# RamSaw/PipelineDP

Hardware: AMD Instinct MI355X
Metric: records/sec DPEngine.aggregate COUNT+SUM at 1/2/4/8 MI355X; % HBM roofline (higher is better)
Workload: dtype f64; 1 GPU; configs[1]: 1e+09 records / 1e+07 privacy ids / 1e+06 Zipf(1.1) partitions per GPU, COUNT+SUM+PRIVACY_ID_COUNT, private partition selection; records_per_gpu=1000000000, privacy_ids_per_gpu=10000000, partitions=1000000, max_partitions_contributed=8, max_contributions_per_partition=2, noise=laplace, selection=truncated_geometric, parallelism=pid-sharded x1, privacy_id_range_supplied=True

## Files before the change

pipelinedp_amd/csrc/dpg_api.hip:

```cpp
#include <dlfcn.h>
#include <hip/hip_runtime.h>
#include <rccl/rccl.h>

#include <algorithm>
#include <cstddef>
#include <chrono>
#include <cmath>
#include <cstdio>
#include <cstdlib>
#include <cstring>
#include <map>
#include <mutex>
#include <string>
#include <thread>
#include <tuple>
#include <vector>

static hipError_t occ_query(int *blocks, const void *kern, int threads, size_t lds) {
    static std::mutex mu;
    static std::map<std::tuple<int, const void *, int, size_t>, int> cache;
    int dev = 0;
    (void)hipGetDevice(&dev);
    std::lock_guard<std::mutex> g(mu);
    const auto key = std::make_tuple(dev, kern, threads, lds);
    const auto it = cache.find(key);
    if (it != cache.end()) {
        *blocks = it->second;
        return hipSuccess;
    }
    const hipError_t e = hipOccupancyMaxActiveBlocksPerMultiprocessor(blocks, kern, threads, lds);
    if (e == hipSuccess) cache[key] = *blocks;
    return e;
}
static hipError_t set_func_attr(const void *kern, hipFuncAttribute attr, int value) {
    if (attr != hipFuncAttributeMaxDynamicSharedMemorySize) return hipFuncSetAttribute(kern, attr, value);
    static std::mutex mu;
    static std::map<std::pair<int, const void *>, int> done;
    int dev = 0;
    (void)hipGetDevice(&dev);
    std::lock_guard<std::mutex> g(mu);
    const auto key = std::make_pair(dev, kern);
    const auto it = done.find(key);
    if (it != done.end() && it->second >= value) return hipSuccess;
    const hipError_t e = hipFuncSetAttribute(kern, attr, value);
    if (e == hipSuccess) done[key] = value;
    return e;
}

#include "dpg_bound.h"
#include "dpg_chunk.h"
#include "dpg_common.h"
#include "dpg_hist.h"
#include "dpg_keydict.h"
#include "dpg_owner.h"
#include "dpg_pairx.h"
#include "dpg_partition.h"
#include "dpg_quantile.h"
#include "dpg_records.h"
#include "dpg_rsort.h"
#include "dpg_sample.h"
#include "dpg_select.h"
#include "dpg_shard.h"
#include "dpg_sortb.h"
#include "dpg_sortmw.h"
#include "dpg_team.h"
#include "dpg_utility.h"
#include "dpg_vsum.h"
#include "dpg_wave.h"
#include "dpg_hist_phases.h"

using namespace dpg;

namespace {

constexpr uint32_t kBucketTarget = 256;
constexpr uint32_t kMaxB1 = 11, kMaxB2 = 12, kMaxBR = 11;
constexpr uint32_t kMaxB1W = 12;
constexpr int kIptL1W = 8;
constexpr uint32_t kPinErr = 4096;
constexpr uint32_t kChunkGroup = 32;
constexpr int kRedoLevel2 = -100;
#ifndef DPG_PC_HALF
#define DPG_PC_HALF 0
#endif
#ifndef DPG_IPT_PC
#define DPG_IPT_PC 8
#endif

struct Buf {
    void *p = nullptr;
    size_t bytes = 0;
};

struct Control {
    uint32_t err;
    uint32_t item_cursor;
    uint32_t ntiles[8];
    int64_t n_scalar;
    uint32_t n_chunks;
    uint32_t n_over;
    uint32_t n_over2;
    uint32_t n_mchunks;
    uint32_t heavy_nfb;
    uint32_t pad_;
    unsigned long long over_records;
    unsigned long long over2_records;
    unsigned long long pid_lo, pid_hi;
};

}

struct dpg_ctx {
    int device = 0;
    uint64_t seed = 0;
    int n_cu = 256;
    std::string err;
    std::map<std::string, Buf> bufs;
    std::vector<std::string> stage_names;
    std::vector<hipEvent_t> events;
    int n_events_used = 0;
    hipStream_t last_stream = nullptr;
    uint32_t bucket_target = 0;
    uint32_t bucket_cap = kBCap;
    void *comm = nullptr;
    const uint32_t *last_err = nullptr;
    int rank = 0, nranks = 1;
    char *stage_buf = nullptr;
    size_t stage_cap = 0, stage_head = 0;
    std::map<hipStream_t, hipEvent_t> stage_done;
    uint32_t *pin_tot = nullptr;
    hipEvent_t tot_ev = nullptr;
    uint32_t team_backoff = 0;
    uint32_t team_backoff_next = 64;
};

namespace {

int watchdog_seconds() {
#if defined(DPG_WATCHDOG) || defined(DPG_PHASE_TIMING)
    const char *e = std::getenv("DPG_WATCHDOG_S");
    return e ? std::atoi(e) : 0;
#else
    return 0;
#endif
}

uint32_t *watchdog_buffer(size_t n) {
    static uint32_t *buf = nullptr;
    static size_t cap = 0;
    if (n > cap) {
        if (buf) (void)hipHostFree(buf);
        if (hipHostMalloc((void **)&buf, n * 4, hipHostMallocCoherent) != hipSuccess) return nullptr;
        cap = n;
    }
    std::memset(buf, 0, n * 4);
    return buf;
}

void watchdog_wait(hipStream_t s, const uint32_t *prog, size_t n, const char *what) {
    int secs = watchdog_seconds();
    for (int i = 0; i < secs * 100; ++i) {
        if (hipStreamQuery(s) == hipSuccess) return;
        std::this_thread::sleep_for(std::chrono::milliseconds(10));
    }
    std::fprintf(stderr, "[dpg watchdog] %s did not finish in %d s; phases:", what, secs);
    for (size_t i = 0; i < n; ++i) std::fprintf(stderr, " %u", prog[i]);
    std::fprintf(stderr, "\n");
    std::fflush(stderr);
    std::abort();
}

int fail(dpg_ctx *c, int code, const std::string &msg) {
    if (c) c->err = msg;
    return code;
}

#define HIP_TRY(expr)                                                                     \
    do {                                                                                  \
        hipError_t e_ = (expr);                                                           \
        if (e_ != hipSuccess)                                                             \
            return fail(ctx, DPG_ERR_HIP, std::string(#expr) + ": " + hipGetErrorString(e_)); \
    } while (0)

#define LAUNCH_CHECK()                                                                        \
    do {                                                                                      \
        hipError_t e_ = hipGetLastError();                                                    \
        if (e_ != hipSuccess)                                                                 \
// ... 779 lines not shown
            for (uint8_t x : hd) nd += x;
            std::fprintf(stderr, "[dpg phase] medium chunks streamed=%u deferred=%zu\n",
                         hctl.n_mchunks, nd);
        }
    }
    if (heavy) {
        HIP_TRY(hipMemcpyAsync(&hctl, ctl, sizeof(Control), hipMemcpyDeviceToHost, s));
        HIP_TRY(hipStreamSynchronize(s));
        const uint32_t nfb = hctl.heavy_nfb;
        if (nfb > 0) {
            WS(fst, int64_t, "heavy.fb.start", nfb);
            WS(fcnt, uint32_t, "heavy.fb.cnt", nfb);
            WS(fd1, uint32_t, "heavy.fb.d1", nfb);
            k_gather_heavy<<<(nfb + 255) / 256, 256, 0, s>>>(hfb, &ctl->heavy_nfb, g_start, g_cnt,
                                                             g_d1, fst, fcnt, fd1);
            LAUNCH_CHECK();
            g_start = fst;
            g_cnt = fcnt;
            g_d1 = fd1;
        }
        if (timing) std::fprintf(stderr, "[dpg phase] heavy buckets=%u handed back=%u\n", n_global, nfb);
        n_global = nfb;
    }
    if (n_global > 0) {
        std::vector<uint32_t> cnt(n_global);
        HIP_TRY(hipMemcpy(cnt.data(), g_cnt, n_global * 4, hipMemcpyDeviceToHost));
        std::vector<size_t> off(n_global);
        size_t total = 0;
        for (uint32_t i = 0; i < n_global; ++i) {
            off[i] = total;
            total += align16(BigLayout::make(cnt[i], ItemTraits<Item>::var).total);
        }
        WS(scratch, char, "bound.scratch", total);
        WS(doff, size_t, "bound.scratch_off", n_global);
        UPLOAD(doff, off.data(), n_global * sizeof(size_t));
        BoundParams bpg = bp;
        uint32_t *gprog = watchdog_seconds() ? watchdog_buffer(n_global) : nullptr;
        bpg.progress = gprog;
        bpg.phase_cyc = timing ? bpl.phase_cyc + 32 : nullptr;
        if (watchdog_seconds())
            std::fprintf(stderr, "[dpg] %u oversize buckets, scratch %zu bytes\n", n_global, total);
        k_bound_big<Item, R><<<n_global, kBigThreads, 0, s>>>(g_base, g_start, g_cnt, g_d1, doff,
                                                              scratch, bpg, items, wg_off + G,
                                                              wg_cnt + G);
        LAUNCH_CHECK();
        if (gprog) watchdog_wait(s, gprog, n_global, "k_bound_big");
        if (timing) {
            unsigned long long h[8];
            HIP_TRY(hipMemcpy(h, bpl.phase_cyc + 32, sizeof(h), hipMemcpyDeviceToHost));
            static const char *nmb[8] = {"clear", "A.insert", "B.slots", "C.mpc", "D.state",
                                         "E.mcpp", "F.acc", "G.emit"};
            unsigned long long tot = 0;
            for (int i = 0; i < 8; ++i) tot += h[i];
            size_t recs_big = 0;
            uint32_t nmax = 0;
            for (uint32_t i = 0; i < n_global; ++i) recs_big += cnt[i], nmax = std::max(nmax, cnt[i]);
            std::fprintf(stderr, "[dpg phase] big buckets=%u records=%zu max=%u per-WG Mcycles:",
                         n_global, recs_big, nmax);
            for (int i = 0; i < 8; ++i)
                std::fprintf(stderr, " %s=%.3f(%.0f%%)", nmb[i], h[i] / 1e6 / n_global,
                             100.0 * h[i] / (tot ? tot : 1));
            std::fprintf(stderr, "\n");
        }
    }
    k_scan_small<<<1, 1024, 0, s>>>(wg_cnt, G + 1, wg_pre, &ctl->item_cursor);
    LAUNCH_CHECK();
    constexpr bool kPA = ItemTraits<Item>::preagg;
    int64_t n_items;
    if constexpr (kPA) {
        HIP_TRY(hipMemcpyAsync(&hctl, ctl, sizeof(Control), hipMemcpyDeviceToHost, s));
        HIP_TRY(hipStreamSynchronize(s));
        if (hctl.err & 2u) return fail(ctx, DPG_ERR_HIP, "internal hash-table error in bounding");
        n_items = hctl.item_cursor;
    } else {
        const uint64_t pairs_per_id = std::max<uint32_t>(1u, per_pid ? bp.L : bp.mpc);
        n_items = (int64_t)std::min<uint64_t>((uint64_t)items_cap,
                                              ((uint64_t)1 << pl.kbits) * pairs_per_id);
    }
    const int64_t P = pl.P;
#ifndef DPG_ITEM_IPT_WIDE
#define DPG_ITEM_IPT_WIDE 4
#endif
    constexpr int kItemIpt = sizeof(Item) == 16 ? 8 : sizeof(Item) == 24 ? DPG_ITEM_IPT_WIDE : 4;
#ifndef DPG_PA_RB
#define DPG_PA_RB 11
#endif
    constexpr uint32_t kRB = kPA ? (uint32_t)DPG_PA_RB : (uint32_t)kRangeBits;
    const int64_t nranges = (P + (1ll << kRB) - 1) >> kRB;
    int64_t *baseR = nullptr;
    uint32_t *totR = nullptr;
    const Item *sorted = items;
    uint32_t F = 1;
    if (n_items > 0) {
        const uint32_t rb = std::max<uint32_t>(1, bits_for((uint64_t)std::max<int64_t>(1, nranges)));
        const uint32_t b2 = rb > 10 ? std::min<uint32_t>(kMaxBR, rb / 2) : 0u;
        const uint32_t b1 = rb - b2;
        const uint32_t F1 = nranges <= 1024 ? (uint32_t)std::max<int64_t>(1, nranges) : 1u << b1;
        WS(items2, Item, "items2", n_items);
        const SrcSeg<Item> src1{items, wg_pre, wg_off, G + 1, kRB + b2};
        int r = run_level<SrcSeg<Item>, Item, kItemIpt, 1024>(
            ctx, s, src1, 1u, nullptr, &ctl->item_cursor, nullptr, n_items, F1, b1, items2,
            "items", &baseR, &totR, &ctl->ntiles[4]);
        if (r) return r;
        sorted = items2;
        F = F1;
        if (b2 > 0) {
            const SrcItems<Item> src2{items2, kRB, (1u << b2) - 1u};
            int64_t *base2;
            uint32_t *tot2;
            r = run_level<SrcItems<Item>, Item, kItemIpt, 2048>(ctx, s, src2, F1, baseR, totR,
                                                                 nullptr, n_items, 1u << b2, b2,
                                                                 items, "items2", &base2, &tot2,
                                                                 &ctl->ntiles[6]);
            if (r) return r;
            baseR = base2;
            totR = tot2;
            sorted = items;
            F = F1 << b2;
        }
    }
    if constexpr (kPA) {
        pa->n_pairs = n_items;
        if (n_items > pa->capacity)
            return fail(ctx, DPG_ERR_INVALID_ARG,
                        "pairs capacity " + std::to_string(pa->capacity) + " < " +
                            std::to_string(n_items) + " pairs");
        if (n_items == 0) {
            HIP_TRY(hipMemsetAsync(pa->partition_start, 0, (P + 1) * 8, s));
            stage(ctx, s, "end");
            return DPG_OK;
        }
        const SrcItems<Item> src3{sorted, 0u, (1u << kRB) - 1u};
        int64_t *base3;
        uint32_t *tot3;
        int r = run_level<SrcItems<Item>, Item, kItemIpt, 2048>(
            ctx, s, src3, F, baseR, totR, nullptr, n_items, 1u << kRB, kRB, pa->pairs, "pairs",
            &base3, &tot3, &ctl->ntiles[7]);
        if (r) return r;
        HIP_TRY(hipMemcpyAsync(pa->partition_start, base3, P * 8, hipMemcpyDeviceToDevice, s));
        k_set_i64<<<1, 1, 0, s>>>(pa->partition_start + P, n_items);
        LAUNCH_CHECK();
    } else if (n_items > 0) {
        Partials po{out->rows, out->count, out->sum, out->nsum, out->nsq};
        stage(ctx, s, "reduce");
        const int64_t rtile = 65536;
        uint32_t max_tiles = (uint32_t)(n_items / rtile + F + 1);
        WS(rt, TileDesc, "reduce.tiles", max_tiles);
        WS(rstb, uint32_t, "reduce.stb", F);
        WS(rsnt, uint32_t, "reduce.snt", F);
        k_build_tiles<<<build_tiles_blocks(F), 256, 0, s>>>(baseR, totR, nullptr, F, rtile, rt, rstb,
                                                      rsnt, &ctl->ntiles[5]);
        LAUNCH_CHECK();
        size_t lds_r = (size_t)kRange * 8 * (ItemTraits<Item>::var ? (ItemTraits<Item>::sum ? 3 : 2) : 1) +
                       kRange * 8;
        k_reduce_items<Item><<<max_tiles, 1024, lds_r, s>>>(sorted, rt, &ctl->ntiles[5], rsnt, P,
                                                         po);
        LAUNCH_CHECK();
    }
    stage(ctx, s, "end");
    return DPG_OK;
}

__global__ void k_region_base(int64_t *rbase, uint32_t F, uint32_t C) {
    const uint32_t i = blockIdx.x * blockDim.x + threadIdx.x;
    if (i >= 8 * F) return;
    const uint32_t x = i / F, d = i % F;
    rbase[i] = ((int64_t)d * 8 + x) * C;
}

__global__ __launch_bounds__(1024) void k_piece_totals(const uint32_t *cum, const int64_t *rbase,
                                                       uint32_t F, uint32_t *tot, uint32_t *ptot,
                                                       int64_t *ostart, PieceDesc *desc) {
    __shared__ uint32_t sh[16];
    constexpr int DPT = 4;
    const uint32_t d0 = DPT * threadIdx.x;
    uint32_t c[DPT], x = 0;
#pragma unroll
    for (int u = 0; u < DPT; ++u) {
        c[u] = 0;
        uint32_t cp = 0;
        if (d0 + u < F) {
            const uint32_t d = d0 + u;
            const int64_t b0 = rbase[d];
            PieceDesc &pd = desc[d];
            for (int r = 0; r < 8; ++r) {
                const uint32_t y = cum[(size_t)r * F + d];
// ... 2181 lines not shown
```

pipelinedp_amd/csrc/dpg_partition.h:

```cpp
#pragma once

#include "dpg_common.h"

#include <type_traits>

namespace dpg {

#ifndef DPG_HIST_U
#define DPG_HIST_U 8
#endif
#ifndef DPG_SCAT_WB
#define DPG_SCAT_WB 2
#endif
constexpr int kPartThreads = 1024;
constexpr int kScatThreads = 1024;

__host__ __device__ constexpr size_t a16(size_t x) { return (x + 15) & ~(size_t)15; }

typedef int64_t i64x2 __attribute__((ext_vector_type(2)));
typedef uint64_t u64x2 __attribute__((ext_vector_type(2)));
typedef uint64_t u64x2a8 __attribute__((ext_vector_type(2), aligned(8)));

template <class Src, class = void>
struct HasFetchPairs {
    static constexpr bool value = false;
};
template <class Src>
struct HasFetchPairs<Src, decltype((void)Src::kFetchPairs)> {
    static constexpr bool value = Src::kFetchPairs;
};

#ifndef DPG_XTILE_PF
#define DPG_XTILE_PF 1
#endif
template <class Src, class = void>
struct HasTilePrefetch {
    static constexpr bool value = false;
};
template <class Src>
struct HasTilePrefetch<Src, decltype((void)Src::kTilePrefetch)> {
    static constexpr bool value = Src::kTilePrefetch && DPG_XTILE_PF;
};

template <class Src, class = void>
struct HasPieces {
    static constexpr bool value = false;
};
template <class Src>
struct HasPieces<Src, decltype((void)Src::kPieces)> {
    static constexpr bool value = Src::kPieces;
};

template <class Src, class = void>
struct HasPairs {
    static constexpr bool value = false;
};
template <class Src>
struct HasPairs<Src, decltype((void)Src::kPairs)> {
    static constexpr bool value = Src::kPairs;
};

struct TileDesc {
    int64_t begin, end;
    uint32_t seg;
    uint32_t pad;
};

__device__ __forceinline__ TileDesc uniform_tile(const TileDesc *tiles, uint32_t t) {
    const TileDesc d = tiles[t];
    auto u64 = [](int64_t x) {
        return (int64_t)(((uint64_t)__builtin_amdgcn_readfirstlane((uint32_t)((uint64_t)x >> 32)) << 32) |
                         (uint32_t)__builtin_amdgcn_readfirstlane((uint32_t)x));
    };
    TileDesc r;
    r.begin = u64(d.begin);
    r.end = u64(d.end);
    r.seg = __builtin_amdgcn_readfirstlane(d.seg);
    r.pad = __builtin_amdgcn_readfirstlane(d.pad);
    return r;
}

template <class R, bool kFull = false>
struct SrcSoAKey {
    static constexpr bool kDigitFromRec = false;
    static constexpr bool kTilePrefetch = true;
    static constexpr bool kPieces = kFull;
    static constexpr bool kV = sizeof(R) == 16;
    using PidW = std::conditional_t<kFull, uint64_t, uint32_t>;
    struct RawK {
        PidW pid;
        int64_t pk;
    };
    struct RawV {
        PidW pid;
        int64_t pk;
        double v;
    };
    using Raw = std::conditional_t<kV, RawV, RawK>;
    const int64_t *pid;
    const int64_t *pk;
    const uint8_t *pub;
    int64_t P;
    int64_t pid_min;
    uint64_t U;
// ... 68 lines not shown
#endif
    static constexpr bool kFetchPairs = DPG_L1_PAIRS != 0;
    __device__ __forceinline__ void fetch2(int64_t i, Raw &x0, Raw &x1) const {
#if DPG_L1_NT
        const u64x2a8 p = __builtin_nontemporal_load(reinterpret_cast<const u64x2a8 *>(pid + i));
        const u64x2a8 q = __builtin_nontemporal_load(reinterpret_cast<const u64x2a8 *>(pk + i));
#else
        const u64x2a8 p = *reinterpret_cast<const u64x2a8 *>(pid + i);
        const u64x2a8 q = *reinterpret_cast<const u64x2a8 *>(pk + i);
#endif
        if constexpr (kV) {
#if DPG_L1_NT
            const u64x2a8 v = __builtin_nontemporal_load(reinterpret_cast<const u64x2a8 *>(value + i));
#else
            const u64x2a8 v = *reinterpret_cast<const u64x2a8 *>(value + i);
#endif
            x0 = Raw{(PidW)p.x, (int64_t)q.x, __builtin_bit_cast(double, v.x)};
            x1 = Raw{(PidW)p.y, (int64_t)q.y, __builtin_bit_cast(double, v.y)};
        } else {
            x0 = Raw{(PidW)p.x, (int64_t)q.x};
            x1 = Raw{(PidW)p.y, (int64_t)q.y};
        }
    }
    static constexpr bool kPairs = true;
    __device__ __forceinline__ bool pairs_ok() const {
        return ((uintptr_t)pid & 15) == 0 && (!pub || ((uintptr_t)pk & 15) == 0);
    }
    __device__ __forceinline__ void hist2(int64_t i, uint32_t (&d)[2], bool (&ok)[2]) const {
        const i64x2 p = *reinterpret_cast<const i64x2 *>(pid + i);
        const uint64_t a0 = (uint64_t)(p.x - pid_min), a1 = (uint64_t)(p.y - pid_min);
        if (a0 >= U || a1 >= U) atomicOr(err, 1u);
        d[0] = hk((uint32_t)a0, H) >> dshift;
        d[1] = hk((uint32_t)a1, H) >> dshift;
        ok[0] = ok[1] = true;
        if (pub) {
            const i64x2 q = *reinterpret_cast<const i64x2 *>(pk + i);
            ok[0] = keep((uint32_t)a0, q.x);
            ok[1] = keep((uint32_t)a1, q.y);
        }
    }
};

template <class R>
struct SrcAoS {
    static constexpr bool kDigitFromRec = true;
    static constexpr bool kTilePrefetch = true;
    using Raw = R;
    const R *a;
    Fmt f;
    uint32_t shift, mask;
    __device__ __forceinline__ R fetch(int64_t i) const { return a[i]; }
    __device__ __forceinline__ uint32_t digit(const R &r) const {
        return (uint32_t)(RecOps<R>::key(r, f) >> shift) & mask;
    }
    __device__ __forceinline__ bool decode(const R &x, int64_t, R &r, uint32_t &d) const {
        r = x;
        d = digit(x);
        return true;
    }
    __device__ __forceinline__ bool hist(int64_t i, uint32_t &d) const {
        d = digit(a[i]);
        return true;
    }
    static constexpr bool kPairs = sizeof(R) == 8;
    static constexpr bool kFetchPairs = sizeof(R) == 8;
    __device__ __forceinline__ void fetch2(int64_t i, R &x0, R &x1) const {
        if constexpr (sizeof(R) == 8) {
            const u64x2a8 w = *reinterpret_cast<const u64x2a8 *>(a + i);
            x0 = R{w.x};
            x1 = R{w.y};
        }
    }
    __device__ __forceinline__ bool pairs_ok() const { return ((uintptr_t)a & 15) == 0; }
    __device__ __forceinline__ void hist2(int64_t i, uint32_t (&d)[2], bool (&ok)[2]) const {
        if constexpr (sizeof(R) == 8) {
            const u64x2 w = *reinterpret_cast<const u64x2 *>(a + i);
            d[0] = digit(R{w.x});
            d[1] = digit(R{w.y});
        }
        ok[0] = ok[1] = true;
    }
};

template <class T>
struct SrcSeg {
    static constexpr bool kDigitFromRec = true;
    using Raw = T;
    const T *a;
    const int64_t *pre;
    const int64_t *off;
    uint32_t S;
    uint32_t shift;
    int64_t lo = 0, hi = 0, base = 0;
    __device__ __forceinline__ T fetch(int64_t i) {
        if (i < lo || i >= hi) {
            uint32_t l = 0, h = S;
            while (h - l > 1) {
                const uint32_t mid = (l + h) >> 1;
                if (pre[mid] <= i) l = mid;
                else h = mid;
            }
            lo = pre[l];
            hi = pre[l + 1];
            base = off[l] - lo;
        }
        return a[base + i];
    }
    __device__ __forceinline__ uint32_t digit(const T &r) const { return r.pk >> shift; }
    __device__ __forceinline__ bool decode(const T &x, int64_t, T &r, uint32_t &d) const {
        r = x;
        d = digit(x);
        return true;
    }
    __device__ __forceinline__ bool hist(int64_t i, uint32_t &d) {
        d = digit(fetch(i));
        return true;
    }
};

template <class T>
struct SrcItems {
    static constexpr bool kDigitFromRec = true;
    using Raw = T;
    const T *a;
    uint32_t shift, mask;
    __device__ __forceinline__ T fetch(int64_t i) const { return a[i]; }
    __device__ __forceinline__ uint32_t digit(const T &r) const { return (r.pk >> shift) & mask; }
    __device__ __forceinline__ bool decode(const T &x, int64_t, T &r, uint32_t &d) const {
        r = x;
        d = digit(x);
        return true;
    }
    __device__ __forceinline__ bool hist(int64_t i, uint32_t &d) const {
        d = digit(a[i]);
        return true;
    }
};

struct XcdQueues {
    uint32_t *q;
    uint32_t *n;
    uint32_t *next;
    uint32_t stride;
};

__global__ void k_build_tiles_single(int64_t n, int64_t tile, uint32_t G, TileDesc *tiles,
                                     uint32_t *seg_tile_base, uint32_t *seg_ntiles,
                                     uint32_t *ntiles_total, XcdQueues xq) {
    const uint32_t nt = (uint32_t)((n + tile - 1) / tile);
    const uint32_t t = blockIdx.x * blockDim.x + threadIdx.x;
    if (t == 0) {
        seg_tile_base[0] = 0;
        seg_ntiles[0] = nt;
        *ntiles_total = nt;
    }
    if (t >= nt) return;
    TileDesc d;
    d.begin = (int64_t)t * tile;
    d.end = min((int64_t)(t + 1) * tile, n);
    d.seg = 0;
    d.pad = 0;
    tiles[t] = d;
    if (!xq.q) return;
    const uint32_t g = t / G, x = g & 7u;
    xq.q[(size_t)x * xq.stride + (g >> 3) * G + t % G] = t;
    atomicAdd(&xq.n[x], 1u);
}

__global__ void k_build_subtiles(const TileDesc *groups, const uint32_t *ngroups, int64_t sub,
                                 TileDesc *tiles, uint32_t *ntiles_total, XcdQueues xq) {
    const uint32_t g = blockIdx.x * blockDim.x + threadIdx.x;
    if (g >= *ngroups) return;
    const TileDesc gd = groups[g];
    const uint32_t nt = (uint32_t)((gd.end - gd.begin + sub - 1) / sub);
    if (!nt) return;
    const uint32_t b = atomicAdd(ntiles_total, nt);
    for (uint32_t j = 0; j < nt; ++j) {
        TileDesc d;
        d.begin = gd.begin + (int64_t)j * sub;
        d.end = min(gd.begin + (int64_t)(j + 1) * sub, gd.end);
        d.seg = gd.seg;
        d.pad = g;
        tiles[b + j] = d;
    }
    const uint32_t x = g & 7u;
    const uint32_t qb = atomicAdd(&xq.n[x], nt);
    for (uint32_t j = 0; j < nt; ++j) xq.q[(size_t)x * xq.stride + qb + j] = b + j;
}

__global__ __launch_bounds__(256) void k_build_tiles(const int64_t *seg_start,
                                                     const uint32_t *seg_cnt,
// ... 8 lines not shown
    if (s >= S) return;
    const int64_t st = seg_start ? seg_start[s] : 0;
    const int64_t n = seg_cnt64 ? seg_cnt64[s] : (int64_t)seg_cnt[s];
    const uint32_t nt = (uint32_t)((n + tile - 1) / tile);
    const uint32_t x = s & 7u;
    uint32_t b = 0, qb = 0;
    if (lane == 0 && nt) {
        b = atomicAdd(ntiles_total, nt);
        if (xq.q) qb = atomicAdd(&xq.n[x], nt);
    }
    b = (uint32_t)__shfl((int)b, 0, 64);
    qb = (uint32_t)__shfl((int)qb, 0, 64);
    if (lane == 0) {
        seg_tile_base[s] = b;
        seg_ntiles[s] = nt;
    }
    for (uint32_t j = lane; j < nt; j += 64) {
        TileDesc d;
        d.begin = st + (int64_t)j * tile;
        d.end = st + min((int64_t)(j + 1) * tile, n);
        d.seg = s;
        d.pad = 0;
        tiles[b + j] = d;
        if (xq.q) xq.q[(size_t)x * xq.stride + qb + j] = b + j;
    }
}

inline uint32_t build_tiles_blocks(uint32_t S) { return (S + 3) / 4; }

template <class Src>
__global__ __launch_bounds__(kPartThreads) void k_hist(Src src_in, const TileDesc *tiles,
                                                       const uint32_t *ntiles, uint32_t F,
                                                       uint32_t *hist) {
    extern __shared__ __attribute__((aligned(16))) uint32_t lh[];
    const uint32_t t = blockIdx.x;
    if (t >= *ntiles) return;
    const TileDesc td = tiles[t];
    const int tid = threadIdx.x;
    const uint32_t copy = (tid >> 6) & 3;
    for (uint32_t d = tid; d < 4 * F; d += kPartThreads) lh[d] = 0;
    __syncthreads();
    uint32_t *my = lh + copy * F;
    Src src = src_in;
    constexpr int U = DPG_HIST_U;
    if constexpr (HasPairs<Src>::value) {
        if (src.pairs_ok()) {
            int64_t b = td.begin;
            const int64_t e = td.end;
            if (b & 1) {
                uint32_t d;
                if (tid == 0 && b < e && src.hist(b, d)) atomicAdd(&my[d], 1u);
                ++b;
            }
            constexpr int U2 = U / 2 > 0 ? U / 2 : 1;
            int64_t i = b + 2 * tid;
            for (; i + 2 * (U2 - 1) * kPartThreads + 1 < e; i += 2 * U2 * kPartThreads) {
                uint32_t d[U2][2];
                bool ok[U2][2];
#pragma unroll
                for (int u = 0; u < U2; ++u) src.hist2(i + 2 * u * kPartThreads, d[u], ok[u]);
#pragma unroll
                for (int u = 0; u < U2; ++u) {
                    if (ok[u][0]) atomicAdd(&my[d[u][0]], 1u);
                    if (ok[u][1]) atomicAdd(&my[d[u][1]], 1u);
                }
            }
            for (; i + 1 < e; i += 2 * kPartThreads) {
                uint32_t d[2];
                bool ok[2];
                src.hist2(i, d, ok);
                if (ok[0]) atomicAdd(&my[d[0]], 1u);
                if (ok[1]) atomicAdd(&my[d[1]], 1u);
            }
            if (i < e) {
                uint32_t d;
                if (src.hist(i, d)) atomicAdd(&my[d], 1u);
            }
            __syncthreads();
            for (uint32_t d = tid; d < F; d += kPartThreads)
                hist[(size_t)t * F + d] = lh[d] + lh[F + d] + lh[2 * F + d] + lh[3 * F + d];
            return;
        }
    }
    int64_t i = td.begin + tid;
    for (; i + (U - 1) * kPartThreads < td.end; i += U * kPartThreads) {
        uint32_t d[U];
        bool ok[U];
#pragma unroll
        for (int u = 0; u < U; ++u) ok[u] = src.hist(i + u * kPartThreads, d[u]);
#pragma unroll
        for (int u = 0; u < U; ++u)
            if (ok[u]) atomicAdd(&my[d[u]], 1u);
    }
    for (; i < td.end; i += kPartThreads) {
        uint32_t d;
        if (src.hist(i, d)) atomicAdd(&my[d], 1u);
    }
    __syncthreads();
    for (uint32_t d = tid; d < F; d += kPartThreads)
        hist[(size_t)t * F + d] = lh[d] + lh[F + d] + lh[2 * F + d] + lh[3 * F + d];
}

__global__ __launch_bounds__(1024) void k_scan_tiles(const uint32_t *seg_tile_base,
                                                     const uint32_t *seg_ntiles, uint32_t F,
                                                     uint32_t *hist, uint32_t *ctot) {
    __shared__ uint32_t part[16][64];
    const uint32_t s = blockIdx.x, c = blockIdx.z, C = gridDim.z;
    const int lane = threadIdx.x & 63, w = threadIdx.x >> 6;
    const uint32_t d = blockIdx.y * 64 + lane;
    const uint32_t nt_all = seg_ntiles[s];
    const uint32_t per = (nt_all + C - 1) / C;
    const uint32_t c0 = min(nt_all, c * per), c1 = min(nt_all, c0 + per);
    const uint32_t nt = c1 - c0, tb = seg_tile_base[s] + c0;
    const uint32_t ch = (nt + 15) / 16;
    const uint32_t t0 = min(nt, w * ch), t1 = min(nt, (w + 1) * ch);
    uint32_t acc = 0;
    if (d < F)
        for (uint32_t t = t0; t < t1; ++t) acc += hist[(size_t)(tb + t) * F + d];
    part[w][lane] = acc;
    __syncthreads();
    uint32_t pre = 0, total = 0;
    for (int k = 0; k < 16; ++k) {
        uint32_t x = part[k][lane];
        if (k < w) pre += x;
        total += x;
    }
    if (d < F) {
        uint32_t run = pre;
        for (uint32_t t = t0; t < t1; ++t) {
            size_t o = (size_t)(tb + t) * F + d;
            uint32_t x = hist[o];
            hist[o] = run;
            run += x;
        }
        if (w == 0) ctot[((size_t)s * C + c) * F + d] = total;
    }
}

__global__ void k_scan_chunks(uint32_t S, uint32_t C, uint32_t F, uint32_t *ctot, uint32_t *tot) {
    const uint32_t i = blockIdx.x * blockDim.x + threadIdx.x;
    if (i >= S * F) return;
    const uint32_t s = i / F, d = i % F;
    uint32_t run = 0;
    for (uint32_t c = 0; c < C; ++c) {
        uint32_t &x = ctot[((size_t)s * C + c) * F + d];
        const uint32_t v = x;
        x = run;
        run += v;
    }
    tot[(size_t)s * F + d] = run;
}

__device__ __forceinline__ uint32_t block_excl_scan_1024(uint32_t x, uint32_t *sh16,
                                                         uint32_t &total) {
    const int lane = threadIdx.x & 63, w = threadIdx.x >> 6;
    uint32_t wt;
    uint32_t e = wave_excl_scan(x, wt);
    if (lane == 63) sh16[w] = wt;
    __syncthreads();
    uint32_t pre = 0, tot = 0;
    for (int k = 0; k < 16; ++k) {
        uint32_t y = sh16[k];
        if (k < w) pre += y;
        tot += y;
    }
    __syncthreads();
// ... 240 lines not shown
        uint64_t bal = __ballot((d >> b) & 1u);
        peers &= ((d >> b) & 1u) ? bal : ~bal;
    }
    const int lane = __lane_id();
    const int leader = peers ? __ffsll((long long)peers) - 1 : lane;
    const uint32_t below = __popcll(peers & ((1ull << lane) - 1ull));
    uint32_t basev = 0;
    if (ok && lane == leader) basev = atomicAdd(&cnt[d], (uint32_t)__popcll(peers));
    basev = __shfl(basev, leader, 64);
    return basev + below;
}

template <class T, int kW = (sizeof(T) % 16 == 0 ? 16 : sizeof(T) % 8 == 0 ? 8 : 4)>
struct Words {
    static constexpr int N = sizeof(T) / 16;
    uint4 w[N];
};
template <class T>
struct Words<T, 8> {
    static constexpr int N = sizeof(T) / 8;
    uint2 w[N];
};
template <class T>
struct Words<T, 4> {
    static constexpr int N = sizeof(T) / 4;
    uint32_t w[N];
};
template <class T>
__device__ __forceinline__ Words<T> to_words(const T &r) {
    Words<T> x;
    __builtin_memcpy(&x, &r, sizeof(T));
    return x;
}
template <class T>
__device__ __forceinline__ T from_words(const Words<T> &x) {
    T r;
    __builtin_memcpy(&r, &x, sizeof(T));
    return r;
}

template <class Src, class Rec, int IPT, int FMAX, int NT = kScatThreads>
constexpr size_t scatter_lds_core() {
    return (size_t)sizeof(Rec) * (NT * IPT + 1) +
           (Src::kDigitFromRec ? 0 : a16((size_t)2 * (NT * IPT + 1))) +
           (size_t)FMAX * 12 + 80;
}
#ifndef DPG_SCAT_LBASE
#define DPG_SCAT_LBASE 1
#endif
#ifndef DPG_PC_NORESET
#define DPG_PC_NORESET 1
#endif
#ifndef DPG_PC_LATE_RSV
#define DPG_PC_LATE_RSV 1
#endif
#ifndef DPG_L1_PF
#define DPG_L1_PF 2
#endif
template <class Src, class Rec, int IPT, int FMAX, int NT = kScatThreads>
constexpr bool scatter_lbase() {
    return scatter_lds_core<Src, Rec, IPT, FMAX, NT>() + (size_t)FMAX * 4 <= 160 * 1024;
}
template <class Src, class Rec, int IPT, int FMAX, int NT = kScatThreads>
constexpr size_t scatter_lds() {
    return scatter_lds_core<Src, Rec, IPT, FMAX, NT>() +
           (scatter_lbase<Src, Rec, IPT, FMAX, NT>() ? (size_t)FMAX * 4 : 0);
}

#ifdef DPG_PHASE_TIMING
__device__ unsigned long long g_scat_cyc[8];
#define DPG_SCAT_MARK(k)                                         \
    do {                                                         \
        if (threadIdx.x == 0) {                                  \
            const uint64_t now_ = __builtin_amdgcn_s_memtime();  \
            scyc[k] += now_ - slast;                             \
            slast = now_;                                        \
        }                                                        \
    } while (0)
#else
#define DPG_SCAT_MARK(k) \
    do {                 \
    } while (0)
#endif

template <class T>
__device__ __forceinline__ const T *uniform_ptr(const T *p) {
    const uint64_t v = (uint64_t)(uintptr_t)p;
    const uint32_t lo = __builtin_amdgcn_readfirstlane((uint32_t)v);
    const uint32_t hi = __builtin_amdgcn_readfirstlane((uint32_t)(v >> 32));
    return reinterpret_cast<const T *>((uintptr_t)(((uint64_t)hi << 32) | lo));
}

template <class Src, class Rec, int IPT, int FMAX, bool kAgg, int NT = kScatThreads>
__global__ __launch_bounds__(NT, 4) void k_scatter(Src src_in, const TileDesc *tiles,
                                                          const uint32_t *ntiles, uint32_t F,
                                                          uint32_t bits, const uint32_t *off,
                                                          const int64_t *base, Rec *out,
                                                          XcdQueues xq = XcdQueues{},
                                                          const uint32_t *cbase = nullptr,
                                                          const uint32_t *seg_tile_base = nullptr,
                                                          const uint32_t *seg_ntiles = nullptr,
                                                          uint32_t C = 1, uint32_t *goff = nullptr,
                                                          uint32_t pcap = 0, uint32_t pdump = 0,
                                                          uint32_t *perr = nullptr) {
    constexpr int SUB = NT * IPT;
    constexpr bool kPc = HasPieces<Src>::value;
    constexpr bool kSD = !Src::kDigitFromRec;
    constexpr bool kP = HasFetchPairs<Src>::value && IPT % 2 == 0;
    constexpr bool kEarly = kPc && kP && DPG_L1_PF != 0;
    constexpr int kPF = kEarly ? DPG_L1_PF : 0;
    using W = Words<Rec>;
    extern __shared__ __attribute__((aligned(16))) char smem[];
    W *stage = reinterpret_cast<W *>(smem);
    uint16_t *sdig = reinterpret_cast<uint16_t *>(smem + sizeof(Rec) * (SUB + 1));
    const size_t o = sizeof(Rec) * (SUB + 1) + (kSD ? a16((size_t)2 * (SUB + 1)) : 0);
    uint32_t *cnt = reinterpret_cast<uint32_t *>(smem + o);
    uint32_t *dstart = cnt + FMAX;
    uint32_t *cur = dstart + FMAX + 1;
    uint32_t *sh16 = cur + FMAX;
    constexpr bool kLB = DPG_SCAT_LBASE && scatter_lbase<Src, Rec, IPT, FMAX, NT>();
    uint32_t *lbase = reinterpret_cast<uint32_t *>(smem + scatter_lds_core<Src, Rec, IPT, FMAX, NT>());
    uint32_t lseg = 0xFFFFFFFFu;

    const uint32_t nt = __builtin_amdgcn_readfirstlane(*ntiles);
    const int tid = threadIdx.x;
    auto elem = [tid](int j) -> uint32_t {
        return kP ? (uint32_t)((j >> 1) * 2 * NT + 2 * tid + (j & 1))
                  : (uint32_t)(j * NT + tid);
    };
    __shared__ uint32_t sh_next;
    const uint32_t xq_id = blockIdx.x & 7u;
    const uint32_t xq_len = xq.q ? __builtin_amdgcn_readfirstlane(xq.n[xq_id]) : 0u;
    constexpr uint32_t kNone = 0xFFFFFFFFu;
    Src src = src_in;
    typename Src::Raw raw[IPT];
    auto load_sub = [&](int64_t b0, uint32_t lim) {
        if constexpr (kEarly) {
#pragma unroll
            for (int m = 0; m < IPT / 2; ++m) {
                const int32_t o = m * 2 * NT + 2 * tid;
                src.fetch2(b0 + min(o, (int32_t)lim - 2), raw[2 * m], raw[2 * m + 1]);
            }
            return;
        } else if constexpr (kP) {
            if (lim >= 2) {
#pragma unroll
                for (int m = 0; m < IPT / 2; ++m) {
                    const uint32_t o = m * 2 * NT + 2 * tid;
                    const uint32_t a = min(o, lim - 2);
                    typename Src::Raw x0, x1;
                    src.fetch2(b0 + a, x0, x1);
                    raw[2 * m] = a == o ? x0 : x1;
                    raw[2 * m + 1] = x1;
                }
                return;
            }
        }
#pragma unroll
        for (int j = 0; j < IPT; ++j) raw[j] = src.fetch(b0 + min(elem(j), lim - 1));
    };
    auto decode_raw = [&](int j, uint32_t lim, int64_t i, Rec &r, uint32_t &d) -> bool {
        if constexpr (kEarly) {
            if ((j & 1) == 0)
                return src.decode((int32_t)elem(j) > (int32_t)lim - 2 ? raw[j + 1] : raw[j], i, r, d);
        }
        return src.decode(raw[j], i, r, d);
    };
    uint32_t it = blockIdx.x;
    uint32_t t = kNone;
    if (xq.q) {
        if (tid == 0) sh_next = atomicAdd(&xq.next[xq_id], 1u);
        __syncthreads();
        const uint32_t w = __builtin_amdgcn_readfirstlane(sh_next);
        if (w < xq_len) t = __builtin_amdgcn_readfirstlane(xq.q[(size_t)xq_id * xq.stride + w]);
    } else if (it < nt) {
        t = it;
    }
    if (t == kNone) return;
#ifdef DPG_PHASE_TIMING
    uint64_t scyc[6] = {0, 0, 0, 0, 0, 0};
    uint64_t slast = __builtin_amdgcn_s_memtime();
#endif
    TileDesc td = uniform_tile(tiles, t);
    const int64_t n_end = kPc ? uniform_tile(tiles, nt - 1).end : 0;
    load_sub(td.begin, (uint32_t)min<int64_t>(SUB, td.end - td.begin));
    constexpr bool kPcLB = kPc && kLB && DPG_PC_NORESET;
    if constexpr (kPcLB) {
        for (uint32_t d = tid; d < F; d += NT) {
            lbase[d] = (uint32_t)base[(size_t)(blockIdx.x & 7u) * F + d];
            cnt[d] = 0;
        }
        __syncthreads();
    }
    for (;;) {
    uint32_t nq = 0;
    const uint32_t *cb = nullptr;
    uint32_t *gof = goff ? goff + (size_t)(kPc ? (blockIdx.x & 7u) : td.pad) * F : nullptr;
    if constexpr (!kPcLB) {
    if (xq.q && tid == 0) nq = atomicAdd(&xq.next[xq_id], 1u);
    __syncthreads();
    if (cbase) {
        const uint32_t nta = seg_ntiles[td.seg], per = (nta + C - 1) / C;
        cb = cbase + ((size_t)td.seg * C + (t - seg_tile_base[td.seg]) / per) * F;
    }
    const uint32_t bsel = kPc ? (blockIdx.x & 7u) : td.seg;
    if (kLB && goff) {
        if (bsel != lseg) {
            for (uint32_t d = tid; d < F; d += NT) lbase[d] = (uint32_t)base[(size_t)bsel * F + d];
            lseg = bsel;
        }
        for (uint32_t d = tid; d < F; d += NT) {
            cur[d] = lbase[d];
            cnt[d] = 0;
        }
    } else {
        for (uint32_t d = tid; d < F; d += NT) {
            cur[d] = (uint32_t)(base[(size_t)bsel * F + d] +
                                (goff ? 0u : off[(size_t)t * F + d] + (cb ? cb[d] : 0u)));
            cnt[d] = 0;
        }
    }
    __syncthreads();
    }
    uint32_t tn = kNone;
    TileDesc tdn = td;
    DPG_SCAT_MARK(4);
    for (int64_t sb = td.begin; sb < td.end; sb += SUB) {
        const uint32_t lim = (uint32_t)min<int64_t>(SUB, td.end - sb);
        Rec rec[IPT];
        uint32_t dr[IPT];
        if constexpr (!kAgg) {
            uint32_t dg[IPT];
            bool okv[IPT];
#pragma unroll
            for (int j = 0; j < IPT; ++j) {
                const uint32_t o = elem(j);
                uint32_t d = 0;
                if constexpr (kEarly)
                    okv[j] = o < lim && decode_raw(j, lim, sb + o, rec[j], d);
                else
                    okv[j] = o < lim && src.decode(raw[j], sb + o, rec[j], d);
                dg[j] = okv[j] ? d : 0u;
            }
            uint32_t rk[IPT];
#pragma unroll
            for (int j = 0; j < IPT; ++j) rk[j] = atomicAdd(&cnt[dg[j]], okv[j] ? 1u : 0u);
#pragma unroll
            for (int j = 0; j < IPT; ++j) dr[j] = okv[j] ? (dg[j] | (rk[j] << 12)) : ~0u;
        } else {
#pragma unroll
            for (int j = 0; j < IPT; ++j) {
                const uint32_t o = elem(j);
                uint32_t d = 0;
                bool ok;
                if constexpr (kEarly)
                    ok = o < lim && decode_raw(j, lim, sb + o, rec[j], d);
                else
                    ok = o < lim && src.decode(raw[j], sb + o, rec[j], d);
                const uint32_t rk = wave_agg_rank(cnt, ok ? d : 0u, ok, bits);
                dr[j] = ok ? (d | (rk << 12)) : ~0u;
            }
        }
        if (xq.q && tid == 0 && sb == td.begin) sh_next = nq;
        __syncthreads();
        DPG_SCAT_MARK(0);
        constexpr int kDPT = FMAX / NT;
        constexpr bool kLate = kPcLB && (kDPT == 2 || kDPT == 4) && FMAX == kDPT * NT && DPG_PC_LATE_RSV;
        PcRsv<(kDPT >= 2 ? kDPT : 2)> rsv;
        uint32_t total;
        if constexpr (!kEarly) {
        if constexpr (kLate)
            total = scatter_scan_pc<NT, kDPT>(cnt, dstart, F, sh16, gof, rsv);
        else
            total = scatter_scan_update<NT, FMAX / NT, kPc>(
                cnt, dstart, cur, F, sh16, gof, pcap, pdump, perr, kPcLB ? lbase : nullptr);
        DPG_SCAT_MARK(1);
        {
            uint32_t ds[IPT];
#pragma unroll
            for (int j = 0; j < IPT; ++j) ds[j] = dstart[dr[j] != ~0u ? (dr[j] & 0xFFFu) : 0u];
#pragma unroll
            for (int j = 0; j < IPT; ++j) {
                const uint32_t pos = dr[j] != ~0u ? ds[j] + (dr[j] >> 12) : (uint32_t)SUB;
                stage[pos] = to_words(rec[j]);
                if constexpr (kSD) sdig[pos] = (uint16_t)(dr[j] & 0xFFFu);
            }
        }
        if constexpr (kLate) scatter_rsv_finish(rsv, cur, lbase, F, pcap, pdump, perr);
        __syncthreads();
        DPG_SCAT_MARK(2);
        const int64_t nb = sb + SUB;
        const uint32_t nlim = (uint32_t)max<int64_t>(0, min<int64_t>(SUB, td.end - nb));
        {
            int64_t lb = nb;
            uint32_t ll = nlim;
            if constexpr (HasTilePrefetch<Src>::value && kPc) {
                if (nlim == 0 && it + gridDim.x < nt) {
                    tn = it + gridDim.x;
                    tdn.begin = (int64_t)tn * SUB;
                    tdn.end = min(tdn.begin + SUB, n_end);
                    lb = tdn.begin;
                    ll = (uint32_t)min<int64_t>(SUB, tdn.end - tdn.begin);
                }
            } else if constexpr (HasTilePrefetch<Src>::value) {
                if (nlim == 0 && xq.q) {
                    const uint32_t w = __builtin_amdgcn_readfirstlane(sh_next);
                    if (w < xq_len) {
                        tn = __builtin_amdgcn_readfirstlane(xq.q[(size_t)xq_id * xq.stride + w]);
                        tdn = uniform_tile(tiles, tn);
                        lb = tdn.begin;
                        ll = (uint32_t)min<int64_t>(SUB, tdn.end - tdn.begin);
                    }
                }
            }
            if (ll > 0) load_sub(lb, ll);
        }
        } else {
        auto prefetch = [&]() {
            const int64_t nb = sb + SUB;
            const uint32_t nlim = (uint32_t)max<int64_t>(0, min<int64_t>(SUB, td.end - nb));
            int64_t lb = nb;
            uint32_t ll = nlim;
            if (nlim == 0) {
                lb = sb;
                ll = lim;
                if (it + gridDim.x < nt) {
                    tn = it + gridDim.x;
                    tdn.begin = (int64_t)tn * SUB;
                    tdn.end = min(tdn.begin + SUB, n_end);
                    lb = tdn.begin;
                    ll = (uint32_t)min<int64_t>(SUB, tdn.end - tdn.begin);
                }
            }
            load_sub(lb, ll);
        };
        if constexpr (kLate && kPF == 3) {
            total = scatter_scan_pc<NT, kDPT>(cnt, dstart, F, sh16, gof, rsv, prefetch);
        } else {
            if constexpr (kLate)
                total = scatter_scan_pc<NT, kDPT>(cnt, dstart, F, sh16, gof, rsv);
            else
                total = scatter_scan_update<NT, FMAX / NT, kPc>(
                    cnt, dstart, cur, F, sh16, gof, pcap, pdump, perr, kPcLB ? lbase : nullptr);
            prefetch();
        }
        DPG_SCAT_MARK(1);
        {
            uint32_t ds[IPT];
#pragma unroll
            for (int j = 0; j < IPT; ++j) ds[j] = dstart[dr[j] != ~0u ? (dr[j] & 0xFFFu) : 0u];
#pragma unroll
            for (int j = 0; j < IPT; ++j) {
                const uint32_t pos = dr[j] != ~0u ? ds[j] + (dr[j] >> 12) : (uint32_t)SUB;
                stage[pos] = to_words(rec[j]);
                if constexpr (kSD) sdig[pos] = (uint16_t)(dr[j] & 0xFFFu);
            }
        }
        if constexpr (kLate) scatter_rsv_finish(rsv, cur, lbase, F, pcap, pdump, perr);
        __syncthreads();
        DPG_SCAT_MARK(2);
        }
        constexpr int WB = IPT < DPG_SCAT_WB ? IPT : DPG_SCAT_WB;
        constexpr int kWbIter = (IPT + WB - 1) / WB;
        auto write_batch = [&](uint32_t k0) {
            W x[WB];
            uint32_t dd[WB], kc[WB];
#pragma unroll
            for (int u = 0; u < WB; ++u) {
                kc[u] = min(k0 + u * NT + tid, total - 1);
                x[u] = stage[kc[u]];
                if constexpr (kSD) dd[u] = sdig[kc[u]];
            }
            if constexpr (!kSD) {
#pragma unroll
                for (int u = 0; u < WB; ++u) dd[u] = src.digit(from_words<Rec>(x[u]));
            }
            uint32_t c1[WB], c2[WB];
#pragma unroll
            for (int u = 0; u < WB; ++u) {
                c1[u] = cur[dd[u]];
                c2[u] = dstart[dd[u] + 1];
            }
#if DPG_EXP_SCAT_NOSTORE
#pragma unroll
            for (int u = 0; u < WB; ++u) {
                uint32_t w0;
                __builtin_memcpy(&w0, &x[u], 4);
                if (w0 == 0x12345u && c1[u] == 0x777u)
                    *reinterpret_cast<W *>(&out[c1[u] - c2[u] + kc[u]]) = x[u];
            }
#else
#pragma unroll
            for (int u = 0; u < WB; ++u) *reinterpret_cast<W *>(&out[c1[u] - c2[u] + kc[u]]) = x[u];
#endif
        };
        if constexpr (kPc) {
#pragma unroll
            for (int b = 0; b < kWbIter; ++b) {
                if ((uint32_t)b * WB * NT >= total) break;
                write_batch((uint32_t)b * WB * NT);
            }
        } else {
            for (uint32_t k0 = 0; k0 < total; k0 += WB * NT) write_batch(k0);
        }
        DPG_SCAT_MARK(3);
#ifdef DPG_PHASE_TIMING
        if (tid == 0) ++scyc[5];
#endif
    }
    if (!HasTilePrefetch<Src>::value && xq.q) {
        const uint32_t w = __builtin_amdgcn_readfirstlane(sh_next);
        if (w >= xq_len) break;
        tn = __builtin_amdgcn_readfirstlane(xq.q[(size_t)xq_id * xq.stride + w]);
        tdn = uniform_tile(tiles, tn);
        load_sub(tdn.begin, (uint32_t)min<int64_t>(SUB, tdn.end - tdn.begin));
    } else if (kPc && HasTilePrefetch<Src>::value) {
        it += gridDim.x;
    } else if (!xq.q) {
        it += gridDim.x;
        if (it >= nt) break;
        tn = it;
        tdn = uniform_tile(tiles, tn);
        load_sub(tdn.begin, (uint32_t)min<int64_t>(SUB, tdn.end - tdn.begin));
    }
    if (tn == kNone) break;
    t = tn;
    td = tdn;
    }
#ifdef DPG_PHASE_TIMING
    if (tid == 0)
        for (int k = 0; k < 6; ++k) atomicAdd(&g_scat_cyc[k], (unsigned long long)scyc[k]);
#endif
}

}
```

Measured before the change: 56.47 billion records/s.

## Resolve segmented item regions per sub-tile with scalar-loaded window and lane permute

Replaces the per-element binary search in SrcSeg fetch with a per-subtile window: the wave finds the starting region with a ballot-based parallel search, scalar-loads eight region bounds and offsets, and each lane picks its base address through a bpermute. This applies to both the histogram and scatter passes of the first items sort level, with a fallback to the old per-element fetch when the window does not cover the subtile. It also changes the items IPT for 16-byte items to 5 and reads and writes staged items as raw vector words in the scatter writeback. The cost it targets is the divergent per-element region lookup. In exchange it adds inline asm, a per-subtile atomic path counter, and a requirement of at least eight regions.

```diff
diff --git a/pipelinedp_amd/csrc/dpg_api.hip b/pipelinedp_amd/csrc/dpg_api.hip
--- a/pipelinedp_amd/csrc/dpg_api.hip
+++ b/pipelinedp_amd/csrc/dpg_api.hip
@@ -103,6 +103,7 @@
     uint32_t n_mchunks;
     uint32_t heavy_nfb;
     uint32_t pad_;
+    uint32_t seg_paths[2];
     unsigned long long over_records;
     unsigned long long over2_records;
     unsigned long long pid_lo, pid_hi;
@@ -1048,6 +1049,10 @@
 #define DPG_ITEM_IPT_WIDE 4
 #endif
     constexpr int kItemIpt = sizeof(Item) == 16 ? 8 : sizeof(Item) == 24 ? DPG_ITEM_IPT_WIDE : 4;
+#ifndef DPG_ITEM_IPT_SEG16
+#define DPG_ITEM_IPT_SEG16 5
+#endif
+    constexpr int kSegIpt = sizeof(Item) == 16 ? DPG_ITEM_IPT_SEG16 : kItemIpt;
 #ifndef DPG_PA_RB
 #define DPG_PA_RB 11
 #endif
@@ -1063,11 +1068,19 @@
         const uint32_t b1 = rb - b2;
         const uint32_t F1 = nranges <= 1024 ? (uint32_t)std::max<int64_t>(1, nranges) : 1u << b1;
         WS(items2, Item, "items2", n_items);
-        const SrcSeg<Item> src1{items, wg_pre, wg_off, G + 1, kRB + b2};
-        int r = run_level<SrcSeg<Item>, Item, kItemIpt, 1024>(
+        if (G + 1 < (uint32_t)kSegK) return fail(ctx, DPG_ERR_HIP, "internal: too few item regions");
+        const SrcSeg<Item> src1{items, wg_pre, wg_off, G + 1, kRB + b2, ctl->seg_paths};
+        int r = run_level<SrcSeg<Item>, Item, kSegIpt, 1024>(
             ctx, s, src1, 1u, nullptr, &ctl->item_cursor, nullptr, n_items, F1, b1, items2,
             "items", &baseR, &totR, &ctl->ntiles[4]);
         if (r) return r;
+        if (std::getenv("DPG_DEBUG_ITEM_PATHS")) {
+            uint32_t hp[2];
+            HIP_TRY(hipMemcpyAsync(hp, ctl->seg_paths, sizeof(hp), hipMemcpyDeviceToHost, s));
+            HIP_TRY(hipStreamSynchronize(s));
+            if (hp[0]) stage(ctx, s, "items.regions=window");
+            if (hp[1]) stage(ctx, s, "items.regions=lookup");
+        }
         sorted = items2;
         F = F1;
         if (b2 > 0) {
diff --git a/pipelinedp_amd/csrc/dpg_partition.h b/pipelinedp_amd/csrc/dpg_partition.h
--- a/pipelinedp_amd/csrc/dpg_partition.h
+++ b/pipelinedp_amd/csrc/dpg_partition.h
@@ -20,6 +20,8 @@
 typedef int64_t i64x2 __attribute__((ext_vector_type(2)));
 typedef uint64_t u64x2 __attribute__((ext_vector_type(2)));
 typedef uint64_t u64x2a8 __attribute__((ext_vector_type(2), aligned(8)));
+typedef uint32_t u32x2 __attribute__((ext_vector_type(2)));
+typedef uint32_t u32x4 __attribute__((ext_vector_type(4)));
 
 template <class Src, class = void>
 struct HasFetchPairs {
@@ -254,16 +256,163 @@
     }
 };
 
+template <class Src, class = void>
+struct HasRegions {
+    static constexpr bool value = false;
+};
+template <class Src>
+struct HasRegions<Src, decltype((void)Src::kRegions)> {
+    static constexpr bool value = Src::kRegions;
+};
+
+constexpr int kSegK = 8;
+
+template <class T>
+__device__ __forceinline__ const T *uniform_ptr(const T *p) {
+    const uint64_t v = (uint64_t)(uintptr_t)p;
+    const uint32_t lo = __builtin_amdgcn_readfirstlane((uint32_t)v);
+    const uint32_t hi = __builtin_amdgcn_readfirstlane((uint32_t)(v >> 32));
+    return reinterpret_cast<const T *>((uintptr_t)(((uint64_t)hi << 32) | lo));
+}
+
+struct SegBounds {
+    int64_t p0, p1, p2, p3, p4, p5, p6, p7, p8;
+    int64_t o0, o1, o2, o3, o4, o5, o6, o7;
+};
+__device__ __forceinline__ SegBounds sload_regions(const int64_t *pre, const int64_t *off) {
+    static_assert(kSegK == 8, "sload_regions lists its loads");
+    int64_t p0, p1, p2, p3, p4, p5, p6, p7, p8, o0, o1, o2, o3, o4, o5, o6, o7;
+    asm volatile(
+        "s_load_dwordx2 %0, %17, 0x0\n\t"
+        "s_load_dwordx2 %1, %17, 0x8\n\t"
+        "s_load_dwordx2 %2, %17, 0x10\n\t"
+        "s_load_dwordx2 %3, %17, 0x18\n\t"
+        "s_load_dwordx2 %4, %17, 0x20\n\t"
+        "s_load_dwordx2 %5, %17, 0x28\n\t"
+        "s_load_dwordx2 %6, %17, 0x30\n\t"
+        "s_load_dwordx2 %7, %17, 0x38\n\t"
+        "s_load_dwordx2 %8, %17, 0x40\n\t"
+        "s_load_dwordx2 %9, %18, 0x0\n\t"
+        "s_load_dwordx2 %10, %18, 0x8\n\t"
+        "s_load_dwordx2 %11, %18, 0x10\n\t"
+        "s_load_dwordx2 %12, %18, 0x18\n\t"
+        "s_load_dwordx2 %13, %18, 0x20\n\t"
+        "s_load_dwordx2 %14, %18, 0x28\n\t"
+        "s_load_dwordx2 %15, %18, 0x30\n\t"
+        "s_load_dwordx2 %16, %18, 0x38\n\t"
+        "s_waitcnt lgkmcnt(0)"
+        : "=&s"(p0), "=&s"(p1), "=&s"(p2), "=&s"(p3), "=&s"(p4), "=&s"(p5), "=&s"(p6), "=&s"(p7),
+          "=&s"(p8), "=&s"(o0), "=&s"(o1), "=&s"(o2), "=&s"(o3), "=&s"(o4), "=&s"(o5), "=&s"(o6),
+          "=&s"(o7)
+        : "s"(pre), "s"(off)
+        : "memory");
+    return SegBounds{p0, p1, p2, p3, p4, p5, p6, p7, p8, o0, o1, o2, o3, o4, o5, o6, o7};
+}
+
+__device__ __forceinline__ int64_t uniform_i64(int64_t x) {
+    return (int64_t)(((uint64_t)__builtin_amdgcn_readfirstlane((uint32_t)((uint64_t)x >> 32)) << 32) |
+                     (uint32_t)__builtin_amdgcn_readfirstlane((uint32_t)x));
+}
+
+struct SegWindow {
+    uint32_t tl, th;
+    uint32_t r1, r2, r3, r4, r5, r6, r7, r8;
+    bool covered;
+};
+
 template <class T>
 struct SrcSeg {
     static constexpr bool kDigitFromRec = true;
+    static constexpr bool kRegions = true;
     using Raw = T;
     const T *a;
     const int64_t *pre;
     const int64_t *off;
     uint32_t S;
     uint32_t shift;
+    uint32_t *paths = nullptr;
     int64_t lo = 0, hi = 0, base = 0;
+    int64_t hint_b = -1;
+    uint32_t hint_l = 0;
+    __device__ __forceinline__ uint32_t find(int64_t b) const {
+        uint32_t l = 0, h = S;
+        const uint32_t lane = __lane_id();
+        while (h - l > 1) {
+            const uint32_t step = (h - l + 63) >> 6;
+            const uint32_t m = l + lane * step;
+            const bool le = m < h && pre[min(m, h - 1)] <= b;
+            const uint32_t c = __builtin_amdgcn_readfirstlane((uint32_t)__popcll(__ballot(le)));
+            h = min(h, l + c * step);
+            l = l + (c - 1) * step;
+        }
+        return l;
+    }
+    __device__ __forceinline__ SegWindow window(int64_t b0, uint32_t lim, int64_t next) {
+        const uint32_t l0 = b0 == hint_b ? hint_l : find(b0);
+        const uint32_t lb = min(l0, S - (uint32_t)kSegK);
+        const SegBounds g = sload_regions(uniform_ptr(pre + lb), uniform_ptr(off + lb));
+        auto addr = [&](int64_t o, int64_t p) { return (uint64_t)(o - p + b0) * sizeof(T); };
+        auto rel = [&](int64_t p) {
+            return (uint32_t)min<int64_t>(max<int64_t>(p - b0, 0), (int64_t)lim);
+        };
+        SegWindow w;
+        const uint64_t ak[kSegK] = {addr(g.o0, g.p0), addr(g.o1, g.p1), addr(g.o2, g.p2),
+                                    addr(g.o3, g.p3), addr(g.o4, g.p4), addr(g.o5, g.p5),
+                                    addr(g.o6, g.p6), addr(g.o7, g.p7)};
+        const uint32_t lane = __lane_id();
+        uint32_t tl = 0, th = 0;
+#pragma unroll
+        for (int k = 0; k < kSegK; ++k) {
+            tl = lane == (uint32_t)k ? (uint32_t)ak[k] : tl;
+            th = lane == (uint32_t)k ? (uint32_t)(ak[k] >> 32) : th;
+        }
+        w.tl = tl;
+        w.th = th;
+        w.r1 = rel(g.p1);
+        w.r2 = rel(g.p2);
+        w.r3 = rel(g.p3);
+        w.r4 = rel(g.p4);
+        w.r5 = rel(g.p5);
+        w.r6 = rel(g.p6);
+        w.r7 = rel(g.p7);
+        w.r8 = rel(g.p8);
+        w.covered = g.p8 - b0 >= (int64_t)lim;
+        auto le = [&](int64_t p) { return p <= next ? 1u : 0u; };
+        const uint32_t k = le(g.p1) + le(g.p2) + le(g.p3) + le(g.p4) + le(g.p5) + le(g.p6) + le(g.p7);
+        hint_b = g.p8 > next ? next : -1;
+        hint_l = lb + k;
+        return w;
+    }
+    __device__ __forceinline__ const char *locate(const SegWindow &w, uint32_t o) const {
+        o = min(o, w.r8 - 1u);
+        const uint32_t k = (o >= w.r1 ? 1u : 0u) + (o >= w.r2 ? 1u : 0u) + (o >= w.r3 ? 1u : 0u) +
+                           (o >= w.r4 ? 1u : 0u) + (o >= w.r5 ? 1u : 0u) + (o >= w.r6 ? 1u : 0u) +
+                           (o >= w.r7 ? 1u : 0u);
+        const uint32_t xl = (uint32_t)__builtin_amdgcn_ds_bpermute((int)(k << 2), (int)w.tl);
+        const uint32_t xh = (uint32_t)__builtin_amdgcn_ds_bpermute((int)(k << 2), (int)w.th);
+        const uint64_t x = ((uint64_t)xh << 32) | xl;
+        return reinterpret_cast<const char *>(a) + (x + (uint64_t)o * sizeof(T));
+    }
+    template <int N, class Pos>
+    __device__ __forceinline__ bool fetch_sub(int64_t b0, uint32_t lim, int64_t next, Pos pos,
+                                              T (&raw)[N]) {
+        const SegWindow w = window(b0, lim, next);
+#pragma unroll
+        for (int j = 0; j < N; ++j) raw[j] = *reinterpret_cast<const T *>(locate(w, pos(j)));
+        asm volatile("" ::: "memory");
+        return w.covered;
+    }
+    template <int N, class Pos>
+    __device__ __forceinline__ bool hist_sub(int64_t b0, uint32_t lim, int64_t next, Pos pos,
+                                             uint32_t (&d)[N]) {
+        const SegWindow w = window(b0, lim, next);
+        uint32_t pk[N];
+#pragma unroll
+        for (int j = 0; j < N; ++j) pk[j] = reinterpret_cast<const T *>(locate(w, pos(j)))->pk;
+#pragma unroll
+        for (int j = 0; j < N; ++j) d[j] = pk[j] >> shift;
+        return w.covered;
+    }
     __device__ __forceinline__ T fetch(int64_t i) {
         if (i < lo || i >= hi) {
             uint32_t l = 0, h = S;
@@ -279,6 +428,8 @@
         return a[base + i];
     }
     __device__ __forceinline__ uint32_t digit(const T &r) const { return r.pk >> shift; }
+    static_assert(offsetof(T, pk) == 0, "the partition key is an item's first word");
+    __device__ __forceinline__ uint32_t digit_word0(uint32_t pk) const { return pk >> shift; }
     __device__ __forceinline__ bool decode(const T &x, int64_t, T &r, uint32_t &d) const {
         r = x;
         d = digit(x);
@@ -453,6 +604,27 @@
             return;
         }
     }
+    if constexpr (HasRegions<Src>::value) {
+        const int64_t tb = uniform_i64(td.begin), te = uniform_i64(td.end);
+        for (int64_t b = tb; b < te; b += U * kPartThreads) {
+            const uint32_t lim = (uint32_t)min<int64_t>(U * kPartThreads, te - b);
+            uint32_t d[U];
+            const bool fast = src.hist_sub(b, lim, b + U * kPartThreads,
+                                           [tid](int u) { return (uint32_t)(u * kPartThreads + tid); }, d);
+            if (!fast) {
+#pragma unroll
+                for (int u = 0; u < U; ++u)
+                    (void)src.hist(b + min((uint32_t)(u * kPartThreads + tid), lim - 1), d[u]);
+            }
+#pragma unroll
+            for (int u = 0; u < U; ++u)
+                if ((uint32_t)(u * kPartThreads + tid) < lim) atomicAdd(&my[d[u]], 1u);
+        }
+        __syncthreads();
+        for (uint32_t d = tid; d < F; d += kPartThreads)
+            hist[(size_t)t * F + d] = lh[d] + lh[F + d] + lh[2 * F + d] + lh[3 * F + d];
+        return;
+    }
     int64_t i = td.begin + tid;
     for (; i + (U - 1) * kPartThreads < td.end; i += U * kPartThreads) {
         uint32_t d[U];
@@ -859,14 +1031,6 @@
     do {                 \
     } while (0)
 #endif
-
-template <class T>
-__device__ __forceinline__ const T *uniform_ptr(const T *p) {
-    const uint64_t v = (uint64_t)(uintptr_t)p;
-    const uint32_t lo = __builtin_amdgcn_readfirstlane((uint32_t)v);
-    const uint32_t hi = __builtin_amdgcn_readfirstlane((uint32_t)(v >> 32));
-    return reinterpret_cast<const T *>((uintptr_t)(((uint64_t)hi << 32) | lo));
-}
 
 template <class Src, class Rec, int IPT, int FMAX, bool kAgg, int NT = kScatThreads>
 __global__ __launch_bounds__(NT, 4) void k_scatter(Src src_in, const TileDesc *tiles,
@@ -911,6 +1075,8 @@
     constexpr uint32_t kNone = 0xFFFFFFFFu;
     Src src = src_in;
     typename Src::Raw raw[IPT];
+    constexpr bool kSeg = HasRegions<Src>::value;
+    bool seg_fast = true;
     auto load_sub = [&](int64_t b0, uint32_t lim) {
         if constexpr (kEarly) {
 #pragma unroll
@@ -932,6 +1098,10 @@
                 }
                 return;
             }
+        }
+        if constexpr (kSeg) {
+            seg_fast = src.fetch_sub(b0, lim, b0 + SUB, elem, raw);
+            return;
         }
 #pragma unroll
         for (int j = 0; j < IPT; ++j) raw[j] = src.fetch(b0 + min(elem(j), lim - 1));
@@ -1006,6 +1176,13 @@
         const uint32_t lim = (uint32_t)min<int64_t>(SUB, td.end - sb);
         Rec rec[IPT];
         uint32_t dr[IPT];
+        if constexpr (kSeg) {
+            if (!seg_fast) {
+#pragma unroll
+                for (int j = 0; j < IPT; ++j) raw[j] = src.fetch(sb + min(elem(j), lim - 1));
+            }
+            if (src.paths && tid == 0) atomicAdd(&src.paths[seg_fast ? 0 : 1], 1u);
+        }
         if constexpr (!kAgg) {
             uint32_t dg[IPT];
             bool okv[IPT];
@@ -1141,14 +1318,28 @@
         constexpr int kWbIter = (IPT + WB - 1) / WB;
         auto write_batch = [&](uint32_t k0) {
             W x[WB];
+            static_assert(!kSeg || sizeof(W) / W::N >= 8, "items are read as 8- or 16-byte words");
+            using NV = std::conditional_t<sizeof(W) / W::N == 16, u32x4, u32x2>;
+            NV xv[WB][W::N];
             uint32_t dd[WB], kc[WB];
 #pragma unroll
             for (int u = 0; u < WB; ++u) {
                 kc[u] = min(k0 + u * NT + tid, total - 1);
-                x[u] = stage[kc[u]];
+                if constexpr (kSeg) {
+#pragma unroll
+                    for (int q = 0; q < W::N; ++q)
+                        xv[u][q] = reinterpret_cast<const NV *>(&stage[kc[u]])[q];
+                } else {
+                    x[u] = stage[kc[u]];
+                }
                 if constexpr (kSD) dd[u] = sdig[kc[u]];
             }
-            if constexpr (!kSD) {
+            if constexpr (kSeg) {
+#pragma unroll
+                for (int u = 0; u < WB; ++u) {
+                    dd[u] = src.digit_word0(xv[u][0].x);
+                }
+            } else if constexpr (!kSD) {
 #pragma unroll
                 for (int u = 0; u < WB; ++u) dd[u] = src.digit(from_words<Rec>(x[u]));
             }
@@ -1168,10 +1359,18 @@
             }
 #else
 #pragma unroll
-            for (int u = 0; u < WB; ++u) *reinterpret_cast<W *>(&out[c1[u] - c2[u] + kc[u]]) = x[u];
+            for (int u = 0; u < WB; ++u) {
+                W *dst = reinterpret_cast<W *>(&out[c1[u] - c2[u] + kc[u]]);
+                if constexpr (kSeg) {
+#pragma unroll
+                    for (int q = 0; q < W::N; ++q) reinterpret_cast<NV *>(dst)[q] = xv[u][q];
+                } else {
+                    *dst = x[u];
+                }
+            }
 #endif
         };
-        if constexpr (kPc) {
+        if constexpr (kPc || kSeg) {
 #pragma unroll
             for (int b = 0; b < kWbIter; ++b) {
                 if ((uint32_t)b * WB * NT >= total) break;
```

After: 57.42 billion records/s (median of 6 runs). +1.7%, better.
